# AustenLamacraft/audio-mps

Measured on AMD Instinct MI355X. Metric: audio samples/sec (fwd+bwd) at D=32, T=16000, higher is better.
Workload: dtype f32; 1 GPU; BASELINE configs[2]: PsiCMPS fwd+bwd scan, D=32, T=16000, batch 1024 per GPU (global 1024), input damped_sine, full optimiser step (device-resident chain rule + Adam); parallelism=dp1, kernel_variant=2, kernel_family=wave, input=damped_sine, optimizer_step=device (cmps_psi_apply_step), rank1_updates=f16x2

## Files before the change

### audio_mps_amd/csrc/cmps_wave_bwd2.hip

```cpp
#include "cmps_wave_util.h"

namespace cmps {

namespace {

struct Pre2 {
    float yh, yho, yhp, un, pre;
    v2f rho;
    v2f sd;
    float inv, ten, rad;
    float q;
};

constexpr int RING_SLOT = 256;
constexpr int RING_VAL = 8 * RING_SLOT;
constexpr int RING_HALF = 3 * RING_VAL;
constexpr int SPIN_MAX = 1 << 22;
constexpr int MT = 4;

__device__ __forceinline__ void flag_store2(unsigned addr_l, int v) {
    asm volatile("ds_write_b32 %0, %1" : : "v"(addr_l), "v"(v) : "memory");
}
__device__ __forceinline__ void swap_fill(float& a, float& b, v2f& m0, v2f r0, v2f q0, v2f& m1, v2f r1, v2f q1, v2f s2) {
    asm("v_pk_fma_f32 %2, %4, %8, %5 op_sel_hi:[1,0,1]\n\t"
        "v_pk_fma_f32 %3, %6, %8, %7 op_sel_hi:[1,0,1]\n\t"
        "v_permlane32_swap_b32 %0, %1"
        : "+v"(a), "+v"(b), "=&v"(m0), "=&v"(m1) : "v"(r0), "v"(q0), "v"(r1), "v"(q1), "v"(s2));
}
__device__ __forceinline__ void own_issue_n(unsigned ay, unsigned ap, unsigned ar, unsigned as, v2f& yh, float& part, v2f& t, v4f& c0) {
    asm volatile("ds_read_b64 %0, %4\n\tds_read_b32 %1, %5\n\tds_read_b64 %2, %6\n\tds_read_b128 %3, %7"
                 : "=&v"(yh), "=&v"(part), "=&v"(t), "=&v"(c0) : "v"(ay), "v"(ap), "v"(ar), "v"(as) : "memory");
}
template <int OY, int OR, int OS>
__device__ __forceinline__ void own_issue_n_off(unsigned ay, unsigned ap, unsigned ar, unsigned as, v2f& yh, float& part, v2f& t, v4f& c0) {
    asm volatile("ds_read_b64 %0, %4 offset:%8\n\tds_read_b32 %1, %5 offset:%8\n\tds_read_b64 %2, %6 offset:%9\n\t"
                 "ds_read_b128 %3, %7 offset:%10"
                 : "=&v"(yh), "=&v"(part), "=&v"(t), "=&v"(c0) : "v"(ay), "v"(ap), "v"(ar), "v"(as), "n"(OY), "n"(OR), "n"(OS)
                 : "memory");
}
template <int N>
__device__ __forceinline__ void lds_wait_own_n(v2f& yh, float& part, v2f& t, v4f& c0) {
    asm volatile("s_waitcnt lgkmcnt(%4)" : "+v"(yh), "+v"(part), "+v"(t), "+v"(c0) : "n"(N) : "memory");
}
template <int OFF>
__device__ __forceinline__ void ring_write(unsigned addr, float v) {
    asm volatile("ds_write_b32 %0, %1 offset:%2" : : "v"(addr), "v"(v), "n"(OFF) : "memory");
}
__device__ __forceinline__ float wave_max(float x) {
    asm("s_nop 1\n\tv_max_f32_dpp %0, %0, %0 quad_perm:[1,0,3,2] row_mask:0xf bank_mask:0xf\n\t"
        "s_nop 1\n\tv_max_f32_dpp %0, %0, %0 quad_perm:[2,3,0,1] row_mask:0xf bank_mask:0xf\n\t"
        "s_nop 1\n\tv_max_f32_dpp %0, %0, %0 row_half_mirror row_mask:0xf bank_mask:0xf\n\t"
        "s_nop 1\n\tv_max_f32_dpp %0, %0, %0 row_mirror row_mask:0xf bank_mask:0xf\n\t"
        "s_nop 1\n\tv_max_f32_dpp %0, %0, %0 row_bcast:15 row_mask:0xa bank_mask:0xf\n\t"
        "s_nop 1\n\tv_max_f32_dpp %0, %0, %0 row_bcast:31 row_mask:0xc bank_mask:0xf" : "+v"(x));
    return rdlane(x, 63);
}

}

template <bool NORM = false>
__global__ __launch_bounds__(128 * WAVES, 1) void k_bwd_wave2w(Dev Pk, const float* __restrict__ audio) {
    const Dev P = NORM ? bank_view(Pk, blockIdx.y) : bank_view_phi(Pk, blockIdx.y);
    audio += blockIdx.y * P.bank_audio;
    __shared__ __attribute__((aligned(16))) float4 stY[WAVES][CHB * 32];
    __shared__ __attribute__((aligned(16))) float4 stR[WAVES][CHB * 16];
    __shared__ __attribute__((aligned(16))) float4 scl[WAVES][CH * 2];
    __shared__ __attribute__((aligned(16))) float2 bcB[WAVES][DPW];
    __shared__ __attribute__((aligned(16))) float ring[WAVES][2 * 3 * 8 * 64];
    __shared__ __attribute__((aligned(8))) float2 sct[WAVES][2][CH];
    __shared__ int flags[WAVES][2];
    __shared__ int flag_sink[WAVES][2][64];
    const int wv = __builtin_amdgcn_readfirstlane(threadIdx.x >> 6), lane = threadIdx.x & 63;
    const int w = wv & (WAVES - 1), role = wv / WAVES;
    const int i = lane & 31, h = lane >> 5;
    const bool hb = h != 0;
    if (threadIdx.x < 2 * WAVES) (&flags[0][0])[threadIdx.x] = 0;
    __syncthreads();
    const int b = blockIdx.x * WAVES + w;
    if (b >= P.B) return;
    const int N = P.N, T = P.T, NC = (N + CH - 1) / CH;
    const int u_top = (N - 1) & 7, a_oct = (N - 1 - u_top) >> 3, n_oct = (u_top ? 1 : 0) + a_oct + 1;
    const unsigned aProd = lds_addr(&flags[w][0]), aCons = lds_addr(&flags[w][1]);
    const unsigned aProdL = lane == 0 ? aProd : lds_addr(&flag_sink[w][0][lane]), aConsL = lane == 0 ? aCons : lds_addr(&flag_sink[w][1][lane]);
    const unsigned aRing0 = lds_addr(&ring[w][0]) + lane * 4;
    const int vr = P.phi0 ? P.phi_rank : 1;
    const int bc = b / vr, av = b - bc * vr;
    const float* xrow = audio + (size_t)bc * T;
    const float* sc = P.scal + scal_off(bc, NC, 0);
    const float A = dev_A(P);
    float* slab = P.slabs + (size_t)b * P.slab_floats;
    constexpr int DD = DPW * DPW;

    if (role == 0) {
        __builtin_amdgcn_s_setprio(3);
        stagger(w);
        v2f MRd[16], MQ[16], MM[16];
#pragma unroll
        for (int m = 0; m < 16; ++m) {
            const v2f rt = ld2(&P.RT[i * DPW + 16 * h + m]);
            MRd[m] = mk2(rt.x, -rt.y);
            MQ[m] = ld2(&P.Q[i * DPW + 16 * h + m]);
        }
        const unsigned aBw = lds_addr(&bcB[w][0]) + i * 8 + h * 4, aBr = lds_addr(&bcB[w][0]) + h * 128;
        const unsigned aYown = lds_addr(&stY[w][0]) + (2 * i + h) * 8;
        const unsigned aYpart = lds_addr(&stY[w][0]) + (2 * i + (1 - h)) * 8;
        const unsigned sgn_h = hb ? 0x80000000u : 0u;
        const unsigned aRho = lds_addr(&stR[w][0]) + i * 8;
        const unsigned aScl = lds_addr(&scl[w][0]);
        const float4* rho4 = reinterpret_cast<const float4*>(P.rho);
        const float4* sty4 = reinterpret_cast<const float4*>(P.hst + wave_row(bc, N, 0, vr, av));
        float facc = 0.f, accS = 0.f, accA = 0.f;
        float ra0 = 0.f, ra1 = 0.f, rdt = 0.f, rnv = 1.f, rev = 0.f;
        float rad_above = 0.f;
        v4f so4[4], so2[2];
        auto octet_load = [&](int hh, int q) {
            stage_load512<4>(sty4, hh * CHB + 8 * q, N - 1, lane, so4, vr);
            stage_load<2>(rho4, hh * CHB + 8 * q, N, lane, so2);
        };
        const unsigned so_lane16 = (unsigned)lane * 16u;
        auto octet_load_below = [&](int hh, int q) {
            if (vr == 1) {
                const int row0 = __builtin_amdgcn_readfirstlane(hh * CHB + 8 * q);
                const float4* py = sty4 + (size_t)row0 * WAVE_ROW_QUADS;
                const float4* pr = rho4 + (size_t)row0 * 16;
                asm volatile("global_load_dwordx4 %0, %6, %7\n\tglobal_load_dwordx4 %1, %6, %7 offset:1024\n\t"
                             "global_load_dwordx4 %2, %6, %7 offset:2048\n\tglobal_load_dwordx4 %3, %6, %7 offset:3072\n\t"
                             "global_load_dwordx4 %4, %6, %8\n\tglobal_load_dwordx4 %5, %6, %8 offset:1024"
                             : "=&v"(so4[0]), "=&v"(so4[1]), "=&v"(so4[2]), "=&v"(so4[3]), "=&v"(so2[0]), "=&v"(so2[1])
                             : "v"(so_lane16), "s"(py), "s"(pr) : "memory");
            } else {
                octet_load(hh, q);
            }
        };
        auto octet_commit = [&](int q) {
            stage_commit<4>(&stY[w][q * 256], lane, so4);
            stage_commit<2>(&stR[w][q * 128], lane, so2);
        };
        auto octet_commit_below = [&](int q) {
            asm volatile("s_waitcnt vmcnt(0)" : "+v"(so4[0]), "+v"(so4[1]), "+v"(so4[2]), "+v"(so4[3]), "+v"(so2[0]), "+v"(so2[1]) : : "memory");
            octet_commit(q);
        };
        auto scal_load = [&](int c) {
            const int idx = c * CH + lane;
            ra0 = idx < T ? xrow[idx] : 0.f;
            ra1 = idx + 1 < T ? xrow[idx + 1] : 0.f;
            rdt = P.dtk[idx];
            rnv = sc[scal_n(c, lane)];
            rev = sc[scal_e(c, lane)];
        };
        auto scal_commit = [&](int c) {
            const int idx = c * CH + lane;
            const float inc = ra1 - ra0;
            const float nv = rnv, ev = rev;
            const float invv = rsq_newton(fmaxf(nv, 1e-12f));
            const float invokv = nv > 1e-12f ? invv : 0.f;
            const float sv = inc / A;
            const float ex = ev * inc;
            const float z = ex / A;
            const float zbar = -1.0f / (1.0f + z);
            const float ebar = zbar * inc / A;
            const float tev = 2.0f * ebar;
            if constexpr (NORM) {
                const float radv = tev * ev;
                float radn = __shfl_down(radv, 1, 64);
                if (lane == CH - 1) radn = rad_above;
                if (idx + 1 >= N) radn = 0.f;
                rad_above = rdlane(radv, 0);
                const bool ok = nv > 1e-12f;
                scl[w][lane] = make_float4(sv, rdt, ok ? invv : -invv, ok ? radn * invv : 0.f);
            } else {
            scl[w][2 * lane] = make_float4(sv, rdt, invv, tev * nv);
            scl[w][2 * lane + 1] = make_float4(tev, invokv, tev * ev, 0.f);
            }
            sct[w][c & 1][lane] = make_float2(sv, tev * nv);
            if (idx < N) accA += zbar * ex;
        };
        auto make_pre = [&](v2f yh2, v2f rho, v4f c0, v4f c1, v2f sfill) -> Pre2 {
            const float yown = yh2.x, hown = yh2.y;
            Pre2 S;
            S.rho = rho;
            S.sd = __builtin_shufflevector(c0, c0, 0, 1);
            S.inv = c0.z;
            S.ten = c0.w;
            const float te = c1.x;
            const float invok = c1.y;
            S.rad = c1.z;
            S.pre = te * hown;
            S.yh = S.inv * yown;
            S.yhp = invok * yown;
            {
                float ya = S.yh, yb = S.yh;
                swap_fill(ya, yb, MM[10], MRd[10], MQ[10], MM[11], MRd[11], MQ[11], sfill);
                S.yho = hb ? -ya : yb;
            }
            const v2f un = cmul2(mk2(S.yh, S.yho), rho);
            S.un = un.x;
            return S;
        };

        auto make_pre_n = [&](v2f yh2, float part, v2f rho, v4f c0) -> Pre2 {
            Pre2 S;
            S.rho = rho;
            S.sd = __builtin_shufflevector(c0, c0, 0, 1);
            S.inv = c0.z;
            S.q = c0.w;
            S.yh = yh2.x;
            S.pre = __builtin_fmaf(-S.q, yh2.x, yh2.y);
            S.yho = __uint_as_float(__float_as_uint(part) ^ sgn_h);
            S.un = __builtin_fmaf(-S.yho, rho.y, S.yh * rho.x);
            return S;
        };

        const int hl = (N - 1) / CHB;
#pragma unroll 1
        for (int q = 0; q < 4; ++q) { octet_load(hl, q); octet_commit(q); }
        scal_load(hl >> 1);
        scal_commit(hl >> 1);
        v4f qc[8];
        v2f yh_j, rho_j;
        v4f c0_j, c1_j;
        float part_j;
        Pre2 S;
        if constexpr (NORM) {
            const int jr = (N - 1) & (CHB - 1), jc = (N - 1) & (CH - 1);
            own_issue_n(aYown + jr * 512, aYpart + jr * 512, aRho + jr * 256, aScl + jc * 16, yh_j, part_j, rho_j, c0_j);
            lds_wait_own_n<0>(yh_j, part_j, rho_j, c0_j);
            S = make_pre_n(yh_j, part_j, rho_j, c0_j);
        } else {
            const int jr = (N - 1) & (CHB - 1), jc = (N - 1) & (CH - 1);
            own_issue(aYown + jr * 512, aRho + jr * 256, aScl + jc * 32, yh_j, rho_j, c0_j, c1_j);
            lds_wait_own<0>(yh_j, rho_j, c0_j, c1_j);
            S = make_pre(yh_j, rho_j, c0_j, c1_j, __builtin_shufflevector(c0_j, c0_j, 0, 1));
        }
        {
            const v2f s2 = mk2(S.sd.x, S.sd.x);
#pragma unroll
            for (int m = 16 - MT; m < 16; ++m) MM[m] = __builtin_elementwise_fma(MRd[m], s2, MQ[m]);
        }
        float g = 0.f, go = 0.f;
        const float2 p0 = P.phi0 ? P.phi0[av * DPW + i] : P.psi0[i];
        const float u0 = hb ? p0.y : p0.x;
        float rad_next = 0.f;

        auto chain_step = [&](const Pre2& S, float uk, auto have_pre, bool exact, unsigned aslot, auto slot_off) -> Pre2 {
            constexpr int SO = decltype(slot_off)::value;
            facc += S.sd.y * (go * S.un);
            const v2f yhbp = cmul2_conj_b(mk2(g, go), S.rho);
            const float yhb = yhbp.x;
            float ybar;
            if constexpr (NORM) {
                ybar = __builtin_fmaf(yhb, __builtin_fabsf(S.inv), S.pre);
                if (exact) {
                    asm volatile("" ::: "memory");
                    const float dsum = sum64(S.yh * yhb);
                    const float okinv = S.inv > 0.f ? S.inv : 0.f;
                    ybar = __builtin_fmaf(__builtin_fmaf(-okinv, dsum, S.q), S.yh, ybar);
                }
            } else {
            float dot = rad_next;
            if (exact) {
                asm volatile("" ::: "memory");
                dot = sum64(S.yhp * yhb);
            }
            rad_next = S.rad;
            ybar = (yhb - dot * S.yhp) * S.inv + S.pre;
            }
            bcast_issue(aBw, aBr, ybar, qc);
            {
                const v2f s2 = mk2(S.sd.x, S.sd.x);
#pragma unroll
                for (int m = 0; m < (NORM ? 16 - MT : 16 - MT - 2); ++m) MM[m] = __builtin_elementwise_fma(MRd[m], s2, MQ[m]);
            }
            Pre2 Sn = S;
            if constexpr (!NORM && !decltype(have_pre)::value) {
                const v2f s2 = mk2(S.sd.x, S.sd.x);
                MM[10] = __builtin_elementwise_fma(MRd[10], s2, MQ[10]);
                MM[11] = __builtin_elementwise_fma(MRd[11], s2, MQ[11]);
            }
            if constexpr (decltype(have_pre)::value) {
                if constexpr (NORM) {
                    lds_wait_own_n<9>(yh_j, part_j, rho_j, c0_j);
                    Sn = make_pre_n(yh_j, part_j, rho_j, c0_j);
                } else {
                    lds_wait_own<9>(yh_j, rho_j, c0_j, c1_j);
                    Sn = make_pre(yh_j, rho_j, c0_j, c1_j, S.sd);
                }
                uk = Sn.un;
            }
            ring_write<SO>(aslot, ybar);
            ring_write<SO + RING_VAL>(aslot, S.yh);
            ring_write<SO + 2 * RING_VAL>(aslot, uk);
            lds_wait_lo<4 + 3>(qc);
            v2f am;
            mv1_lo(MM, qc, am);
            lds_wait_hi<3>(qc);
            mv1_hi(MM, qc, am);
            const v2f sn2 = __builtin_shufflevector(c0_j, c0_j, 0, 1);
            float sx = am.x, sy = am.y;
            swap_fill(sx, sy, MM[12], MRd[12], MQ[12], MM[13], MRd[13], MQ[13], sn2);
            const float md = sx + sy;
            accS += md * uk;
            g = ybar + md;
            float ga = g, gb = g;
            swap_fill(ga, gb, MM[14], MRd[14], MQ[14], MM[15], MRd[15], MQ[15], sn2);
            go = hb ? -ga : gb;
            return Sn;
        };
        int oct = 0;
        auto half_base = [&](int o) { return aRing0 + (unsigned)(o & 1) * RING_HALF; };
        int cons_seen = 0;
        auto peek_cons = [&]() {
            asm volatile("ds_read_b32 %0, %1" : "=v"(cons_seen) : "v"(aCons) : "memory");
        };
        auto wait_free = [&](int o) {
            int seen;
            asm volatile("s_nop 0\n\tv_readfirstlane_b32 %0, %1" : "=s"(seen) : "v"(cons_seen));
            if (o >= 2 && seen < o - 1) {
                int spin = 0;
                while (flag_load(aCons) < o - 1 && ++spin < SPIN_MAX) __builtin_amdgcn_s_sleep(1);
            }
        };
        auto publish = [&]() {
            ++oct;
            flag_store2(aProdL, oct);
        };

        const bool proj_ok = P.phi0 == nullptr;
        if (hl >= 1) {
            const int jtop = N - 2, q_hi = jtop >= hl * CHB ? (jtop & (CHB - 1)) >> 3 : -1;
#pragma unroll 1
            for (int q = q_hi + 1; q < 4; ++q) { octet_load(hl - 1, q); octet_commit(q); }
        }
        if (u_top) {
            const unsigned ab = half_base(0);
            for (int t = 0; t < 8 - u_top; ++t) {
                asm volatile("ds_write_b32 %0, %1\n\tds_write_b32 %0, %1 offset:%2\n\tds_write_b32 %0, %1 offset:%3"
                             : : "v"(ab + t * RING_SLOT), "v"(0.f), "n"(RING_VAL), "n"(2 * RING_VAL) : "memory");
            }
        }
        for (int hh = hl; hh >= 0; --hh) {
            const int jlo = hh * CHB;
            const int jhi = (N - 2) < (jlo + CHB - 1) ? (N - 2) : (jlo + CHB - 1);
            const bool new_scal = (hh & 1) == 0 && hh > 0;
            if (new_scal) scal_load((hh >> 1) - 1);
            int j = jhi;
            if (j >= jlo && (j & 7) != 7) {
                const unsigned ab = half_base(0);
                const int q = (j & (CHB - 1)) >> 3;
                if (hh > 0) octet_load(hh - 1, q);
                int t = 8 - u_top;
                for (; j >= jlo && (j & 7) != 7; --j, ++t) {
                    const int jr = j & (CHB - 1), jc = j & (CH - 1);
                    if constexpr (NORM) own_issue_n(aYown + jr * 512, aYpart + jr * 512, aRho + jr * 256, aScl + jc * 16, yh_j, part_j, rho_j, c0_j);
                    else own_issue(aYown + jr * 512, aRho + jr * 256, aScl + jc * 32, yh_j, rho_j, c0_j, c1_j);
                    S = chain_step(S, 0.f, std::true_type{}, proj_ok && j == jhi, ab + t * RING_SLOT, std::integral_constant<int, 0>{});
                }
                if (hh > 0) octet_commit(q);
                publish();
            }
#define BWD2_STEP8(PQ)                                                                                         \
            {                                                                                                 \
                if ((PQ) == 3) peek_cons();                                                                                \
                if constexpr (NORM) own_issue_n_off<(PQ) * 512, (PQ) * 256, (PQ) * 16>(aYo8, aPo8, aRo8, aSo8, yh_j, part_j, rho_j, c0_j);   \
                else own_issue_off<(PQ) * 512, (PQ) * 256, (PQ) * 32>(aYo8, aRo8, aSo8, yh_j, rho_j, c0_j, c1_j);  \
                S = chain_step(S, 0.f, std::true_type{}, (PQ) == 7 && proj_ok && j == jhi, ab8, std::integral_constant<int, (7 - (PQ)) * RING_SLOT>{}); \
            }
            for (; j >= jlo; j -= 8) {
                const int q = (j & (CHB - 1)) >> 3;
                if (hh > 0) octet_load_below(hh - 1, q);
                wait_free(oct);
                const unsigned ab8 = half_base(oct);
                const unsigned aYo8 = aYown + ((j - 7) & (CHB - 1)) * 512, aRo8 = aRho + ((j - 7) & (CHB - 1)) * 256;
                const unsigned aSo8 = aScl + ((j - 7) & (CH - 1)) * (NORM ? 16 : 32);
                const unsigned aPo8 = aYpart + ((j - 7) & (CHB - 1)) * 512;
                BWD2_STEP8(7) BWD2_STEP8(6) BWD2_STEP8(5) BWD2_STEP8(4) BWD2_STEP8(3) BWD2_STEP8(2) BWD2_STEP8(1) BWD2_STEP8(0)
                if (hh > 0) octet_commit_below(q);
                publish();
            }
#undef BWD2_STEP8
            if (new_scal) scal_commit((hh >> 1) - 1);
        }
        {
            wait_free(oct);
            const unsigned ab = half_base(oct);
            S = chain_step(S, u0, std::false_type{}, proj_ok, ab, std::integral_constant<int, 0>{});
            for (int t = 1; t < 8; ++t) {
                asm volatile("ds_write_b32 %0, %1\n\tds_write_b32 %0, %1 offset:%2\n\tds_write_b32 %0, %1 offset:%3"
                             : : "v"(ab + t * RING_SLOT), "v"(0.f), "n"(RING_VAL), "n"(2 * RING_VAL) : "memory");
            }
            publish();
        }
        const float sumS = sum64(accS);
        const float sumA = av == 0 ? sum64(accA) : 0.f;
        const float ftot = swap32_add(facc, facc);
        slab[4 * DD + (hb ? 2 * DPW : DPW) + i] = g;
        if (!hb) slab[4 * DD + i] = ftot;
        if (lane == 0) {
            slab[4 * DD + 3 * DPW] = -(sumA / (A * A)) - sumS / A;
            slab[4 * DD + 3 * DPW + 1] = 0.f;
        }
        return;
    }

    __builtin_amdgcn_s_setprio(0);
    v16f Rre = {}, Rim = {}, Qre = {}, Qim = {};
    constexpr float SB16 = 8192.f;
    float sR = 1.f, sQ = 1.f;
    auto pow2_of = [](float bound) {
        int se = 12 - ((int)((__float_as_uint(bound) >> 23) & 0xFFu) - 126);
        se = se > 60 ? 60 : se < -60 ? -60 : se;
        return __uint_as_float((unsigned)(127 + se) << 23);
    };
    auto pow2_inv = [](float s2) { return __uint_as_float(0x7F000000u - __float_as_uint(s2)); };
    const unsigned aPart = lds_addr(&ring[w][0]) + (lane ^ 32) * 4;
    const unsigned aSct0 = lds_addr(&sct[w][0][0]);
    for (int o = 0; o < n_oct; ++o) {
        {
            int spin = 0;
            while (flag_load(aProd) < o + 1 && ++spin < SPIN_MAX) __builtin_amdgcn_s_sleep(2);
        }
        const unsigned ab = aRing0 + (unsigned)(o & 1) * RING_HALF, ap = aPart + (unsigned)(o & 1) * RING_HALF;
        const int ktop = (u_top && o == 0) ? (N - 1) + (8 - u_top) : (o == n_oct - 1) ? 0 : (N - 1 - u_top) - 8 * (o - (u_top ? 1 : 0));
        int kl = ktop - (lane & 7);
        kl = kl < 0 ? 0 : (kl > N - 1 ? N - 1 : kl);
        const unsigned aSct = aSct0 + (unsigned)(((kl >> 6) & 1) * CH + (kl & (CH - 1))) * 8;
        float yb[8], yh[8], yhq[8], uu[8], uq[8];
        v2f stv;
#pragma unroll
        for (int t = 0; t < 8; t += 2) {
            asm volatile("ds_read2st64_b32 %0, %5 offset0:%7 offset1:%8\n\tds_read2st64_b32 %1, %5 offset0:%9 offset1:%10\n\t"
                         "ds_read2st64_b32 %2, %6 offset0:%9 offset1:%10\n\tds_read2st64_b32 %3, %5 offset0:%11 offset1:%12\n\t"
                         "ds_read2st64_b32 %4, %6 offset0:%11 offset1:%12"
                         : "=&v"(*reinterpret_cast<v2f*>(&yb[t])), "=&v"(*reinterpret_cast<v2f*>(&yh[t])), "=&v"(*reinterpret_cast<v2f*>(&yhq[t])),
                           "=&v"(*reinterpret_cast<v2f*>(&uu[t])), "=&v"(*reinterpret_cast<v2f*>(&uq[t]))
                         : "v"(ab), "v"(ap), "n"(t), "n"(t + 1), "n"(8 + t), "n"(8 + t + 1), "n"(16 + t), "n"(16 + t + 1) : "memory");
        }
        asm volatile("ds_read_b64 %0, %1" : "=&v"(stv) : "v"(aSct) : "memory");
        asm volatile("s_waitcnt lgkmcnt(0)" : "+v"(yb[0]), "+v"(yb[1]), "+v"(yb[2]), "+v"(yb[3]), "+v"(yb[4]), "+v"(yb[5]), "+v"(yb[6]), "+v"(yb[7]) :: "memory");
        asm volatile("s_waitcnt lgkmcnt(0)" : "+v"(yh[0]), "+v"(yh[1]), "+v"(yh[2]), "+v"(yh[3]), "+v"(yh[4]), "+v"(yh[5]), "+v"(yh[6]), "+v"(yh[7]) :: "memory");
        asm volatile("s_waitcnt lgkmcnt(0)" : "+v"(yhq[0]), "+v"(yhq[1]), "+v"(yhq[2]), "+v"(yhq[3]), "+v"(yhq[4]), "+v"(yhq[5]), "+v"(yhq[6]), "+v"(yhq[7]) :: "memory");
        asm volatile("s_waitcnt lgkmcnt(0)" : "+v"(uu[0]), "+v"(uu[1]), "+v"(uu[2]), "+v"(uu[3]), "+v"(uu[4]), "+v"(uu[5]), "+v"(uu[6]), "+v"(uu[7]) :: "memory");
        asm volatile("s_waitcnt lgkmcnt(0)" : "+v"(uq[0]), "+v"(uq[1]), "+v"(uq[2]), "+v"(uq[3]), "+v"(uq[4]), "+v"(uq[5]), "+v"(uq[6]), "+v"(uq[7]), "+v"(stv) :: "memory");
        flag_store2(aConsL, o + 1);
        float a1[8], a2[8], mQ = 0.f, mR = 0.f;
#pragma unroll
        for (int t = 0; t < 8; ++t) {
            const float sk = rdlane(stv.x, t), tn = rdlane(stv.y, t);
            a1[t] = tn * yh[t];
            a2[t] = sk * yb[t];
            mQ = fmaxf(mQ, fabsf(yb[t]));
            mR = fmaxf(mR, fmaxf(fabsf(a1[t]), fabsf(a2[t])));
        }
        mQ = wave_max(mQ);
        mR = wave_max(mR);
        {
            const float xq = mQ * sQ, xr = mR * sR;
            const bool chQ = mQ > 0.f && !(xq >= 32.f && xq < 32768.f), chR = mR > 0.f && !(xr >= 32.f && xr < 32768.f);
            if (chQ || chR) {
                const float nQ = chQ ? pow2_of(mQ) : sQ, nR = chR ? pow2_of(mR) : sR;
                const float fQ = nQ * pow2_inv(sQ), fR = nR * pow2_inv(sR);
#pragma unroll
                for (int r = 0; r < 16; ++r) { Rre[r] *= fR; Rim[r] *= fR; Qre[r] *= fQ; Qim[r] *= fQ; }
                sQ = nQ; sR = nR;
            }
        }
        unsigned fH[7][4], fL[7][4];
        auto split_pair = [&](int v, int reg, float ve, float vo, float sc2) {
            const v2f t = mk2(ve, vo) * mk2(sc2, sc2);
            const h2 hh = {(_Float16)t.x, (_Float16)t.y};
            const unsigned H = __builtin_bit_cast(unsigned, hh);
            float re, ro;
            asm("v_fma_mix_f32 %0, %2, %4, -%5 op_sel:[0,0,0] op_sel_hi:[0,0,1]\n\t"
                "v_fma_mix_f32 %1, %3, %4, -%5 op_sel:[0,0,1] op_sel_hi:[0,0,1]"
                : "=&v"(re), "=&v"(ro) : "v"(ve), "v"(vo), "v"(sc2), "v"(H));
            const h2 ll = {(_Float16)re, (_Float16)ro};
            fH[v][reg] = H;
            fL[v][reg] = __builtin_bit_cast(unsigned, ll);
        };
        const float sgB = hb ? -SB16 : SB16;
#pragma unroll
        for (int r = 0; r < 4; ++r) {
            split_pair(0, r, a1[2 * r], a1[2 * r + 1], sR);
            split_pair(1, r, yb[2 * r], yb[2 * r + 1], sQ);
            split_pair(2, r, a2[2 * r], a2[2 * r + 1], sR);
            split_pair(3, r, yh[2 * r], yh[2 * r + 1], SB16);
            split_pair(4, r, yhq[2 * r], yhq[2 * r + 1], sgB);
            split_pair(5, r, uu[2 * r], uu[2 * r + 1], SB16);
            split_pair(6, r, uq[2 * r], uq[2 * r + 1], sgB);
        }
        auto frag = [&](const unsigned (&f)[4]) { return __builtin_bit_cast(h8, v4u{f[0], f[1], f[2], f[3]}); };
        auto mf3 = [&](v16f& acc, int ia, int ib) {
            acc = __builtin_amdgcn_mfma_f32_32x32x16_f16(frag(fH[ia]), frag(fH[ib]), acc, 0, 0, 0);
            acc = __builtin_amdgcn_mfma_f32_32x32x16_f16(frag(fH[ia]), frag(fL[ib]), acc, 0, 0, 0);
            acc = __builtin_amdgcn_mfma_f32_32x32x16_f16(frag(fL[ia]), frag(fH[ib]), acc, 0, 0, 0);
        };
        mf3(Rre, 0, 3);
        mf3(Rim, 0, 4);
        mf3(Qre, 1, 5);
        mf3(Qim, 1, 6);
        mf3(Rre, 2, 5);
        mf3(Rim, 2, 6);
    }
    const float uR = pow2_inv(sR) * (1.0f / SB16), uQ = pow2_inv(sQ) * (1.0f / SB16);
#pragma unroll
    for (int r = 0; r < 16; ++r) {
        const int row = (r & 3) + 8 * (r >> 2) + 4 * h;
        const int oo = row * DPW + i;
        slab[oo] = Rre[r] * uR;
        slab[DD + oo] = -Rim[r] * uR;
        slab[2 * DD + oo] = Qre[r] * uQ;
        slab[3 * DD + oo] = -Qim[r] * uQ;
    }
}

hipError_t launch_bwd_wave2w(const Dev& P, const float* audio, hipStream_t s, int M) {
    const unsigned nb = (unsigned)((P.B + WAVES - 1) / WAVES);
    if (P.stash_layout == STASH_WAVE32N) hipLaunchKernelGGL(k_bwd_wave2w<true>, dim3(nb, M), dim3(128 * WAVES), 0, s, P, audio);
    else hipLaunchKernelGGL(k_bwd_wave2w<false>, dim3(nb, M), dim3(128 * WAVES), 0, s, P, audio);
    return hipGetLastError();
}

}
```

Baseline: 1.747 billion samples/s.

## Add fully unrolled full-chunk NORM backward path with fused chain tail asm

For the NORM variant, this adds a specialised path for full chunks when vr==1. It unrolls all four octets with compile-time LDS offsets and issues global loads at precomputed addresses, so per-step address arithmetic and branching go away. It also fuses the chain step's tail (the permlane swaps, adds and sign select via a ballot mask) into one inline-asm block using hard-coded v254/v255, and rewrites a few multiply-adds as explicit FMAs. The hard-coded registers and the changed rounding (fmaf versus mul+add, made conditional) could cause register conflicts or numerical drift.

Result: faster. 1.783 billion samples/s (median of 6 runs) (+2.1%).

```diff
diff --git a/audio_mps_amd/csrc/cmps_wave_bwd2.hip b/audio_mps_amd/csrc/cmps_wave_bwd2.hip
--- a/audio_mps_amd/csrc/cmps_wave_bwd2.hip
+++ b/audio_mps_amd/csrc/cmps_wave_bwd2.hip
@@ -27,6 +27,23 @@
         "v_permlane32_swap_b32 %0, %1"
         : "+v"(a), "+v"(b), "=&v"(m0), "=&v"(m1) : "v"(r0), "v"(q0), "v"(r1), "v"(q1), "v"(s2));
 }
+__device__ __forceinline__ void chain_tail_n(v2f am, float ybar, unsigned long long hmask, float& md, float& g, float& go,
+                                             v2f& m0, v2f r0, v2f q0, v2f& m1, v2f r1, v2f q1, v2f& m2, v2f r2, v2f q2, v2f& m3, v2f r3, v2f q3,
+                                             v2f s2) {
+    asm("v_pk_fma_f32 %3, %8, %16, %9 op_sel_hi:[1,0,1]\n\t"
+        "v_pk_fma_f32 %4, %10, %16, %11 op_sel_hi:[1,0,1]\n\t"
+        "v_permlane32_swap_b32 v254, v255\n\t"
+        "v_add_f32 %0, v254, v255\n\t"
+        "v_add_f32 v254, %17, %0\n\t"
+        "v_add_f32 v255, %17, %0\n\t"
+        "v_pk_fma_f32 %5, %12, %16, %13 op_sel_hi:[1,0,1]\n\t"
+        "v_pk_fma_f32 %6, %14, %16, %15 op_sel_hi:[1,0,1]\n\t"
+        "v_permlane32_swap_b32 v254, v255\n\t"
+        "v_cndmask_b32_e64 %1, v254, v255, %18\n\t"
+        "v_cndmask_b32_e64 %2, v255, -v254, %18"
+        : "=&v"(md), "=&v"(g), "=&v"(go), "=&v"(m0), "=&v"(m1), "=&v"(m2), "=&v"(m3), "+{v[254:255]}"(am)
+        : "v"(r0), "v"(q0), "v"(r1), "v"(q1), "v"(r2), "v"(q2), "v"(r3), "v"(q3), "v"(s2), "v"(ybar), "s"(hmask));
+}
 __device__ __forceinline__ void own_issue_n(unsigned ay, unsigned ap, unsigned ar, unsigned as, v2f& yh, float& part, v2f& t, v4f& c0) {
     asm volatile("ds_read_b64 %0, %4\n\tds_read_b32 %1, %5\n\tds_read_b64 %2, %6\n\tds_read_b128 %3, %7"
                  : "=&v"(yh), "=&v"(part), "=&v"(t), "=&v"(c0) : "v"(ay), "v"(ap), "v"(ar), "v"(as) : "memory");
@@ -45,6 +62,10 @@
 template <int OFF>
 __device__ __forceinline__ void ring_write(unsigned addr, float v) {
     asm volatile("ds_write_b32 %0, %1 offset:%2" : : "v"(addr), "v"(v), "n"(OFF) : "memory");
+}
+__device__ __forceinline__ float mul_add_rounded(float a, float b, float c) {
+#pragma clang fp contract(off)
+    return a * b + c;
 }
 __device__ __forceinline__ float wave_max(float x) {
     asm("s_nop 1\n\tv_max_f32_dpp %0, %0, %0 quad_perm:[1,0,3,2] row_mask:0xf bank_mask:0xf\n\t"
@@ -105,6 +126,7 @@
         const unsigned aYown = lds_addr(&stY[w][0]) + (2 * i + h) * 8;
         const unsigned aYpart = lds_addr(&stY[w][0]) + (2 * i + (1 - h)) * 8;
         const unsigned sgn_h = hb ? 0x80000000u : 0u;
+        const unsigned long long hmask = __builtin_amdgcn_ballot_w64(hb);
         const unsigned aRho = lds_addr(&stR[w][0]) + i * 8;
         const unsigned aScl = lds_addr(&scl[w][0]);
         const float4* rho4 = reinterpret_cast<const float4*>(P.rho);
@@ -131,6 +153,13 @@
             } else {
                 octet_load(hh, q);
             }
+        };
+        auto octet_load_at = [&](const float4* py, const float4* pr) {
+            asm volatile("global_load_dwordx4 %0, %6, %7\n\tglobal_load_dwordx4 %1, %6, %7 offset:1024\n\t"
+                         "global_load_dwordx4 %2, %6, %7 offset:2048\n\tglobal_load_dwordx4 %3, %6, %7 offset:3072\n\t"
+                         "global_load_dwordx4 %4, %6, %8\n\tglobal_load_dwordx4 %5, %6, %8 offset:1024"
+                         : "=&v"(so4[0]), "=&v"(so4[1]), "=&v"(so4[2]), "=&v"(so4[3]), "=&v"(so2[0]), "=&v"(so2[1])
+                         : "v"(so_lane16), "s"(py), "s"(pr) : "memory");
         };
         auto octet_commit = [&](int q) {
             stage_commit<4>(&stY[w][q * 256], lane, so4);
@@ -244,9 +273,16 @@
 
         auto chain_step = [&](const Pre2& S, float uk, auto have_pre, bool exact, unsigned aslot, auto slot_off) -> Pre2 {
             constexpr int SO = decltype(slot_off)::value;
+            if constexpr (NORM) facc = __builtin_fmaf(S.sd.y, go * S.un, facc);
+            else
             facc += S.sd.y * (go * S.un);
-            const v2f yhbp = cmul2_conj_b(mk2(g, go), S.rho);
-            const float yhb = yhbp.x;
+            float yhb;
+            if constexpr (NORM) {
+                yhb = __builtin_fmaf(go, S.rho.y, g * S.rho.x);
+            } else {
+                const v2f yhbp = cmul2_conj_b(mk2(g, go), S.rho);
+                yhb = yhbp.x;
+            }
             float ybar;
             if constexpr (NORM) {
                 ybar = __builtin_fmaf(yhb, __builtin_fabsf(S.inv), S.pre);
@@ -266,6 +302,7 @@
             ybar = (yhb - dot * S.yhp) * S.inv + S.pre;
             }
             bcast_issue(aBw, aBr, ybar, qc);
+            if constexpr (NORM) asm volatile("" : "+v"(facc), "+v"(accS));
             {
                 const v2f s2 = mk2(S.sd.x, S.sd.x);
 #pragma unroll
@@ -296,6 +333,13 @@
             lds_wait_hi<3>(qc);
             mv1_hi(MM, qc, am);
             const v2f sn2 = __builtin_shufflevector(c0_j, c0_j, 0, 1);
+            if constexpr (NORM) {
+                float md;
+                chain_tail_n(am, ybar, hmask, md, g, go, MM[12], MRd[12], MQ[12], MM[13], MRd[13], MQ[13], MM[14], MRd[14], MQ[14],
+                             MM[15], MRd[15], MQ[15], sn2);
+                accS = decltype(have_pre)::value ? mul_add_rounded(md, uk, accS) : __builtin_fmaf(md, uk, accS);
+                return Sn;
+            }
             float sx = am.x, sy = am.y;
             swap_fill(sx, sy, MM[12], MRd[12], MQ[12], MM[13], MRd[13], MQ[13], sn2);
             const float md = sx + sy;
@@ -343,6 +387,35 @@
             const int jhi = (N - 2) < (jlo + CHB - 1) ? (N - 2) : (jlo + CHB - 1);
             const bool new_scal = (hh & 1) == 0 && hh > 0;
             if (new_scal) scal_load((hh >> 1) - 1);
+            if constexpr (NORM) {
+                if (hh > 0 && vr == 1 && jhi == jlo + CHB - 1) {
+                    const unsigned abE = half_base(oct), abO = half_base(oct + 1);
+                    unsigned aSclC;
+                    asm volatile("v_mov_b32 %0, %1" : "=v"(aSclC) : "s"(aScl + (unsigned)(hh & 1) * (CHB * 16)));
+                    const float4* pyC = sty4 + (size_t)(jlo - CHB) * WAVE_ROW_QUADS;
+                    const float4* prC = rho4 + (size_t)(jlo - CHB) * 16;
+#define BWD2_CSTEP(Q, PQ, EX, AB)                                                                                    \
+                    {                                                                                                 \
+                        if ((PQ) == 3) peek_cons();                                                                   \
+                        own_issue_n_off<(8 * (Q) + (PQ)) * 512, (8 * (Q) + (PQ)) * 256, (8 * (Q) + (PQ)) * 16>(aYown, aYpart, aRho, aSclC, yh_j, part_j, rho_j, c0_j); \
+                        S = chain_step(S, 0.f, std::true_type{}, EX, AB, std::integral_constant<int, (7 - (PQ)) * RING_SLOT>{}); \
+                    }
+#define BWD2_COCTET(Q, EX, AB)                                                                                        \
+                    {                                                                                                 \
+                        octet_load_at(pyC + (Q) * 8 * WAVE_ROW_QUADS, prC + (Q) * 8 * 16);                            \
+                        wait_free(oct);                                                                               \
+                        BWD2_CSTEP(Q, 7, EX, AB) BWD2_CSTEP(Q, 6, false, AB) BWD2_CSTEP(Q, 5, false, AB) BWD2_CSTEP(Q, 4, false, AB) \
+                        BWD2_CSTEP(Q, 3, false, AB) BWD2_CSTEP(Q, 2, false, AB) BWD2_CSTEP(Q, 1, false, AB) BWD2_CSTEP(Q, 0, false, AB) \
+                        octet_commit_below(Q);                                                                        \
+                        publish();                                                                                    \
+                    }
+                    BWD2_COCTET(3, proj_ok, abE) BWD2_COCTET(2, false, abO) BWD2_COCTET(1, false, abE) BWD2_COCTET(0, false, abO)
+#undef BWD2_COCTET
+#undef BWD2_CSTEP
+                    if (new_scal) scal_commit((hh >> 1) - 1);
+                    continue;
+                }
+            }
             int j = jhi;
             if (j >= jlo && (j & 7) != 7) {
                 const unsigned ab = half_base(0);
```
